# edshkim98/LocalDiffusion-Hallucination

Measured on AMD Instinct MI355X. Metric: local patches/sec (256^2, T=1000), higher is better.
Workload: dtype bf16; 1 GPU; cfg3: 8 local patches (vertical band masks) of one 3x256x256 image per GPU, 4-stage dim-32 conditional UNet (12.1M params), DDPM T=1000, pred_x0, sigmoid schedule; patches_per_gpu=8, parallelism=patch-sharded x1, one all-gather per sample, step_graph_replay=True, whole_batch_graph_flag=False, concurrent_sub_batches=2, weight_split_levels=0

## Files before the change

### include/localdiff_hip.h

```cpp
#ifndef LOCALDIFF_HIP_H
#define LOCALDIFF_HIP_H

#include <stddef.h>
#include <stdint.h>

#ifdef __cplusplus
extern "C" {
#endif

#define LD_OK 0
#define LD_EINVAL (-1)
#define LD_EHIP (-2)
#define LD_ETIMEOUT (-3)

#define LD_F32 0
#define LD_BF16 1
#define LD_F16 2

#define LD_STAT_STRIPES 16

#define LD_ACT_NONE 0
#define LD_ACT_SILU 1
#define LD_ACT_RELU 2

// ... 115 lines not shown
  ld_src a;
  ld_src b;
  int32_t final_act;
  int32_t pool;
  void* out;
  int32_t B, H, W;
  const int32_t* t_ptr;
  int32_t dtype;
} ld_gn_apply_args;
int ld_gn_apply(const ld_gn_apply_args* args, void* stream);

int ld_linattn_kmax(const void* qkv, uint32_t* kmax_enc, int B, int n, int heads, int dim_head,
                    int dtype, void* stream);
int ld_linattn_ctx(const void* qkv, const uint32_t* kmax_enc, float* ctx_part,
                   int B, int n, int heads, int dim_head, int nchunks, int dtype, void* stream);
int ld_linattn_ctx_reduce(const float* ctx_part, int nchunks, float* ctxn, int B, int heads,
                          int dim_head, void* stream);
int ld_linattn_fold(const float* ctxn, const float* w_out ,
                    void* w_packed , int B, int C, int heads, int dim_head,
                    int perm, int dtype, void* stream);
int ld_linattn_ctxfold(const float* ctx_part, int nchunks, const float* w_out ,
                       void* w_packed , int B, int C, int heads, int dim_head,
                       int perm, int dtype, void* stream);
int ld_linattn_kvctx(const void* x, const void* wkv_packed, const float* kshift, float* ctx_part, int B,
                     int n, int C, int heads, int dim_head, int nchunks, int dtype, void* stream);
int ld_linattn_out(const void* x, const void* wq_packed, const float* qshift, const void* mfold,
                   const float* bias, const float* g2, void* out, int B, int n, int C, float q_scale,
                   int dtype, void* stream);
int ld_linattn_kvctx_terms(const void* x, const void* wkv_packed, const float* kshift, float* ctx_part, int B, int n, int C,
                           int heads, int dim_head, int nchunks, int dtype, int weight_terms, void* stream);
int ld_linattn_out_terms(const void* x, const void* wq_packed, const float* qshift, const void* mfold, const float* bias,
                         const float* g2, void* out, int B, int n, int C, float q_scale, int dtype, int weight_terms,
                         void* stream);
size_t ld_linattn_ctx_part_floats(int B, int heads, int dim_head, int nchunks);

int ld_attention(const void* qkv, void* out, int B, int n, int heads, int dim_head, int dtype,
                 void* stream);

int ld_time_mlp(const int32_t* times, int n, const float* freqs, int dim, const float* w1,
                const float* b1, const float* w2, const float* b2, int time_dim, float* temb,
                void* stream);
int ld_time_mlp_fourier(const int32_t* times, int n, const float* weights, int learned_dim, const float* w1,
                        const float* b1, const float* w2, const float* b2, int time_dim, float* temb, void* stream);
int ld_film(const float* temb, int n, int time_dim, const float* w, const float* b, int two_c,
            float* film, void* stream);

int ld_final_conv(const void* x, const float* w , const float* b, float* out_nchw,
                  int B, int H, int W, int Cin, int Cout, int dtype, void* stream);

int ld_final_step(const void* x, const float* w, const float* b, float* model_out, float* x_t, float* x0_out,
                  const float* sched, const int32_t* t_ptr, float lo, float hi, int objective, uint64_t seed,
                  int64_t noise_stream, int B, int H, int W, int Cin, int Cout, int dtype, void* stream);


int ld_final_step_at(const void* x, const float* w, const float* b, float* model_out, float* x_t, float* x0_out,
                     const float* sched, const int32_t* t_ptr, float lo, float hi, int objective, uint64_t seed,
                     int64_t noise_base, int64_t noise_tmul, int64_t noise_first, const float* keep_mask,
                     int B, int H, int W, int Cin, int Cout, int dtype, void* stream);

#define LD_OBJ_X0 0
#define LD_OBJ_NOISE 1
#define LD_OBJ_V 2
#define LD_SCHED_COLS 8
#define LD_SCHED_COEF1 0
#define LD_SCHED_COEF2 1
#define LD_SCHED_SIGMA 2
// ... 131 lines not shown
```

### localdiffusion-hallucination_amd/_cabi.py

```python
import ctypes as C
import os

from .tuning import lib_override_path

_HERE = os.path.dirname(os.path.abspath(__file__))

LIB_PATH = lib_override_path() or os.path.join(_HERE, "csrc", "liblocaldiff_hip.so")

LD_F32, LD_BF16, LD_F16 = 0, 1, 2
ACT_NONE, ACT_SILU, ACT_RELU = 0, 1, 2
EPI_PLAIN, EPI_QKV_LINEAR, EPI_QKV_FULL, EPI_RMS_RES, EPI_RES, EPI_GN_TAIL = 0, 1, 2, 3, 4, 5
OBJ = {"pred_x0": 0, "pred_noise": 1, "pred_v": 2}
SCHED_COLS = 8
STAT_STRIPES = 16
COUNTER_CONV3X3_C32, COUNTER_CONV3X3_GENERIC, COUNTER_CONV3X3_S32 = 0, 1, 2
SEG_SRC_PLAIN, SEG_SRC_POOL, SEG_SRC_CAT_D2S = 0, 1, 2

vp, i32, i64, u64, f32 = C.c_void_p, C.c_int32, C.c_int64, C.c_uint64, C.c_float


class Src(C.Structure):
    _fields_ = [("data", vp), ("C", i32), ("pix_stride", i32), ("upsample", i32), ("gn_stats", vp),
                ("gn_gamma", vp), ("gn_beta", vp), ("gn_groups", i32), ("act", i32), ("film", vp),
                ("film_tstride", i32), ("film_bstride", i32)]
# ... 47 lines not shown
    "ld_memset_bytes": (C.c_int, [vp, C.c_int, C.c_size_t, vp]),
    "ld_event_create": (C.c_int, [C.POINTER(vp)]),
    "ld_event_record": (C.c_int, [vp, vp]),
    "ld_event_elapsed_ms": (C.c_int, [vp, vp, C.POINTER(f32)]),
    "ld_event_destroy": (C.c_int, [vp]),
    "ld_stream_wait_event": (C.c_int, [vp, vp]),
    "ld_counter": (C.c_longlong, [C.c_int]),
    "ld_tuning_set": (C.c_int, [C.c_char_p, C.c_longlong]),
    "ld_tuning_get": (C.c_int, [C.c_char_p, C.POINTER(C.c_longlong)]),
    "ld_tuning_count": (C.c_int, []),
    "ld_tuning_name": (C.c_char_p, [C.c_int]),
    "ld_range_push": (C.c_int, [C.c_char_p]),
    "ld_range_pop": (C.c_int, []),
    "ld_conv3x3": (C.c_int, [C.POINTER(Conv3x3Args), vp]),
    "ld_conv1x1": (C.c_int, [C.POINTER(Conv1x1Args), vp]),
    "ld_pack_conv_weight": (C.c_int, [vp, vp, vp, C.c_int, C.c_int, C.c_int, C.c_int, C.c_int, vp]),
    "ld_pack_conv_weight_terms": (C.c_int, [vp, vp, vp, C.c_int, C.c_int, C.c_int, C.c_int, C.c_int, C.c_int, vp]),
    "ld_conv_image": (C.c_int, [vp, vp, vp, vp, vp, C.c_int, C.c_int, C.c_int, C.c_int, C.c_int,
                                C.c_int, C.c_int, vp]),
    "ld_stem_packed_bytes": (C.c_size_t, []),
    "ld_pack_stem_weight": (C.c_int, [vp, vp, C.c_int, vp]),
    "ld_conv_stem": (C.c_int, [vp, vp, vp, vp, C.c_int, C.c_int, C.c_int, C.c_int, C.c_int, vp]),
    "ld_conv_stem_begin": (C.c_int, [vp, vp, vp, vp, C.c_int, C.c_int, C.c_int, C.c_int, C.c_int, C.POINTER(StepBeginArgs), vp]),
    "ld_gn_apply": (C.c_int, [C.POINTER(GnApplyArgs), vp]),
    "ld_linattn_kmax": (C.c_int, [vp, vp, C.c_int, C.c_int, C.c_int, C.c_int, C.c_int, vp]),
    "ld_linattn_ctx": (C.c_int, [vp, vp, vp, C.c_int, C.c_int, C.c_int, C.c_int, C.c_int, C.c_int, vp]),
    "ld_linattn_ctx_reduce": (C.c_int, [vp, C.c_int, vp, C.c_int, C.c_int, C.c_int, vp]),
    "ld_linattn_fold": (C.c_int, [vp, vp, vp, C.c_int, C.c_int, C.c_int, C.c_int, C.c_int, C.c_int, vp]),
    "ld_linattn_ctxfold": (C.c_int, [vp, C.c_int, vp, vp, C.c_int, C.c_int, C.c_int, C.c_int, C.c_int, C.c_int, vp]),
    "ld_linattn_kvctx": (C.c_int, [vp, vp, vp, vp, C.c_int, C.c_int, C.c_int, C.c_int, C.c_int, C.c_int, C.c_int, vp]),
    "ld_linattn_out": (C.c_int, [vp, vp, vp, vp, vp, vp, vp, C.c_int, C.c_int, C.c_int, f32, C.c_int, vp]),
    "ld_linattn_kvctx_terms": (C.c_int, [vp, vp, vp, vp, C.c_int, C.c_int, C.c_int, C.c_int, C.c_int, C.c_int, C.c_int, C.c_int, vp]),
    "ld_linattn_out_terms": (C.c_int, [vp, vp, vp, vp, vp, vp, vp, C.c_int, C.c_int, C.c_int, f32, C.c_int, C.c_int, vp]),
    "ld_linattn_ctx_part_floats": (C.c_size_t, [C.c_int, C.c_int, C.c_int, C.c_int]),
    "ld_attention": (C.c_int, [vp, vp, C.c_int, C.c_int, C.c_int, C.c_int, C.c_int, vp]),
    "ld_time_mlp": (C.c_int, [vp, C.c_int, vp, C.c_int, vp, vp, vp, vp, C.c_int, vp, vp]),
    "ld_time_mlp_fourier": (C.c_int, [vp, C.c_int, vp, C.c_int, vp, vp, vp, vp, C.c_int, vp, vp]),
    "ld_film": (C.c_int, [vp, C.c_int, C.c_int, vp, vp, C.c_int, vp, vp]),
    "ld_final_conv": (C.c_int, [vp, vp, vp, vp, C.c_int, C.c_int, C.c_int, C.c_int, C.c_int, C.c_int, vp]),
    "ld_final_step": (C.c_int, [vp, vp, vp, vp, vp, vp, vp, vp, f32, f32, C.c_int, u64, i64, C.c_int, C.c_int, C.c_int,
                                C.c_int, C.c_int, C.c_int, vp]),
    "ld_final_step_at": (C.c_int, [vp, vp, vp, vp, vp, vp, vp, vp, f32, f32, C.c_int, u64, i64, i64, i64, vp, C.c_int,
                                   C.c_int, C.c_int, C.c_int, C.c_int, C.c_int, vp]),
    "ld_timing_begin": (C.c_int, [C.c_int]),
    "ld_timing_count": (C.c_int, []),
    "ld_timing_end": (C.c_int, [vp, C.c_int, vp]),
    "ld_timing_end_abs": (C.c_int, [vp, vp, C.c_int, vp]),
    "ld_randn": (C.c_int, [vp, i64, u64, i64, i64, vp, vp]),
    "ld_randn_at": (C.c_int, [vp, i64, i64, u64, i64, i64, vp, vp]),
    "ld_step_add": (C.c_int, [vp, C.c_int, vp]),
    "ld_step_begin": (C.c_int, [vp, C.c_size_t, vp, C.c_size_t, vp, C.c_int, vp, vp, vp]),
    "ld_step_begin_film": (C.c_int, [vp, C.c_size_t, vp, C.c_size_t, vp, C.c_int, vp, vp, vp, C.c_int, vp, vp]),
    "ld_ddim_step_at": (C.c_int, [vp, vp, vp, vp, vp, vp, f32, f32, C.c_int, i64, vp]),
    "ld_ddpm_step": (C.c_int, [vp, vp, vp, vp, vp, vp, vp, f32, f32, C.c_int, i64, vp]),
    "ld_posterior_step": (C.c_int, [vp, vp, vp, vp, vp, vp, i64, vp]),
    "ld_ddim_step": (C.c_int, [vp, vp, vp, vp, f32, f32, f32, f32, f32, f32, f32, f32, f32, C.c_int,
                               C.c_int, i64, vp]),
    "ld_branch_conditions": (C.c_int, [vp, vp, vp, vp, f32, C.c_int, C.c_int, C.c_int, vp]),
    "ld_mask_out": (C.c_int, [vp, vp, f32, C.c_int, C.c_int, C.c_int, vp]),
    "ld_fuse_ddpm": (C.c_int, [vp, vp, vp, vp, vp, vp, vp, f32, f32, C.c_int, C.c_int, C.c_int, vp]),
    "ld_branch_conditions_k": (C.c_int, [vp, vp, vp, f32, C.c_int, C.c_int, C.c_int, C.c_int, vp]),
    "ld_fuse_ddpm_k": (C.c_int, [vp, vp, vp, vp, vp, vp, vp, f32, f32, C.c_int, C.c_int, C.c_int, C.c_int, vp]),
    "ld_fuse_ddim": (C.c_int, [vp, vp, vp, vp, vp, vp, vp, f32, f32, f32, f32, f32, f32, f32, C.c_int,
                               C.c_int, C.c_int, vp]),
    "ld_fuse_ddim_k": (C.c_int, [vp, vp, vp, vp, vp, vp, vp, f32, f32, f32, f32, f32, f32, f32, C.c_int, C.c_int,
                                 C.c_int, C.c_int, vp]),
# ... 85 lines not shown
```

### localdiffusion-hallucination_amd/csrc/linattn_fused.hip

```cpp
#include "common.hip.h"
#include <stdlib.h>

typedef __attribute__((ext_vector_type(4))) short s16x4;

namespace {
constexpr int CTX_STRIDE = 32 * 32 + 64;
constexpr int KTN = 256;
constexpr int PROW = 96;

__device__ __forceinline__ uint2 tr8(const char* p) {
  s16x4 v = __builtin_amdgcn_ds_read_tr16_b64_v4i16((__attribute__((address_space(3))) s16x4*)(const_cast<char*>(p)));
  return __builtin_bit_cast(uint2, v);
}

struct KvCtxArgs {
  const void* x;
  const uint4* wkv;
  float* ctx_part;
  int n, C, heads, nchunks;
  const float* kshift;
  int wsplit;
};
#define KVCTX_PARAMS const void* x_, const uint4* wkv_, float* ctx_part_, int n_, int C_, int heads_, int nchunks_, const float* kshift_, int wsplit_
#define KVCTX_ARGS(a) (a).x, (a).wkv, (a).ctx_part, (a).n, (a).C, (a).heads, (a).nchunks, (a).kshift, (a).wsplit
// ... 469 lines not shown
      for (int m2 = 0; m2 < MT2; ++m2)
        mma16<T>(o[m2], *reinterpret_cast<const uint4*>(s_mf + (s * MT2 + m2) * 1024 + lane * 16), B2[s]);
    float ss = 0.f;
    float y[MT2][4];
#pragma unroll
    for (int m2 = 0; m2 < MT2; ++m2) {
      const float4 bv = bvr[m2];
      y[m2][0] = o[m2][0] + bv.x; y[m2][1] = o[m2][1] + bv.y; y[m2][2] = o[m2][2] + bv.z; y[m2][3] = o[m2][3] + bv.w;
#pragma unroll
      for (int r = 0; r < 4; ++r) ss = fmaf(y[m2][r], y[m2][r], ss);
    }
    ss = kq4_sum(ss);
    const float inv = rms_rinv<false>(ss);
    {
      static_assert(MT2 % 2 == 0, "m-tiles are stored in pairs");
      char* opix = reinterpret_cast<char*>(reinterpret_cast<T*>(a.out) + ((size_t)b * n + (valid ? p : 0)) * C);
#pragma unroll
      for (int m2 = 0; m2 < MT2; m2 += 2) {
        float r4[2][4];
#pragma unroll
        for (int mm = 0; mm < 2; ++mm) {
          const int mq = m2 + mm;
          const float4 gv = gvr[mq];
          float xr[4];
          load4<T>(reinterpret_cast<const T*>(s_x + ((mq >> 1) * 4 + (mq & 1) * 2 + (kq >> 1)) * PLANE + qq * 16 + (kq & 1) * 8), xr);
          r4[mm][0] = y[mq][0] * inv * gv.x + xr[0]; r4[mm][1] = y[mq][1] * inv * gv.y + xr[1];
          r4[mm][2] = y[mq][2] * inv * gv.z + xr[2]; r4[mm][3] = y[mq][3] * inv * gv.w + xr[3];
        }
        const uint4 w16 = pair_frag16<T>(r4[0], r4[1]);
        if (valid) store16_out(opix + m2 * 16 * sizeof(T) + pair_frag16_off(kq), w16);
      }
    }
  }
  }
}

template <typename T>
int kvctx_launch(const KvCtxArgs& a, int B, hipStream_t st) {
  const int nch = a.C / 32, heads = a.heads, nchunks = a.nchunks;
  const float* kshift = a.kshift;
#ifdef LD_DEBUG_VARIANTS
  static const int no_wph = getenv("LD_KVCTX_V1") ? 1 : 0;
#else
  constexpr int no_wph = 0;
#endif
  if (heads == 4 && (!no_wph || kshift)) {
    const size_t lds2 = (size_t)nch * 4 * KTN * 16 + KTN * sizeof(float);
    dim3 grid2(nchunks, B);
    if (a.wsplit) {
      LD_REQUIRE(nch <= 2, "ld_linattn_kvctx: two-term weights are built for C = 32 / 64 (got %d)", a.C);
      if (nch == 1) {
        if (kshift) LD_LAUNCH((kvctx_wph_kernel<T, 1, true, 1>), grid2, dim3(256), lds2, st, KVCTX_ARGS(a));
        else LD_LAUNCH((kvctx_wph_kernel<T, 1, false, 1>), grid2, dim3(256), lds2, st, KVCTX_ARGS(a));
      } else {
        if (kshift) LD_LAUNCH((kvctx_wph_kernel<T, 2, true, 1>), grid2, dim3(256), lds2, st, KVCTX_ARGS(a));
        else LD_LAUNCH((kvctx_wph_kernel<T, 2, false, 1>), grid2, dim3(256), lds2, st, KVCTX_ARGS(a));
      }
    } else if (nch == 1) {
      if (kshift) LD_LAUNCH((kvctx_wph_kernel<T, 1, true>), grid2, dim3(256), lds2, st, KVCTX_ARGS(a));
      else LD_LAUNCH((kvctx_wph_kernel<T, 1, false>), grid2, dim3(256), lds2, st, KVCTX_ARGS(a));
    } else if (nch == 2) {
      if (kshift) LD_LAUNCH((kvctx_wph_kernel<T, 2, true>), grid2, dim3(256), lds2, st, KVCTX_ARGS(a));
      else LD_LAUNCH((kvctx_wph_kernel<T, 2, false>), grid2, dim3(256), lds2, st, KVCTX_ARGS(a));
    } else {
      if (kshift) LD_HIP(ld_allow_lds((kvctx_wph_kernel<T, 4, true>), lds2));
      else LD_HIP(ld_allow_lds((kvctx_wph_kernel<T, 4, false>), lds2));
// ... 9 lines not shown
  if (nch == 1) {
    LD_LAUNCH((kvctx_kernel<T, 1>), grid, dim3(256), lds, st, KVCTX_ARGS(a));
  } else if (nch == 2) {
    LD_HIP(ld_allow_lds((kvctx_kernel<T, 2>), lds));
    LD_LAUNCH((kvctx_kernel<T, 2>), grid, dim3(256), lds, st, KVCTX_ARGS(a));
  } else {
    LD_HIP(ld_allow_lds((kvctx_kernel<T, 4>), lds));
    LD_LAUNCH((kvctx_kernel<T, 4>), grid, dim3(256), lds, st, KVCTX_ARGS(a));
  }
  LD_LAUNCH_CHECK("linattn_kvctx");
  return LD_OK;
}

template <typename T>
int linout_launch(const LinOutArgs& a, int B, hipStream_t st) {
  const int n = a.n, nch = a.C / 32;
  dim3 grid((n + 128 * LINOUT_TPB - 1) / (128 * LINOUT_TPB), B);
  const size_t lds = (size_t)nch * 4 * 128 * 16 + ((size_t)nch << a.wsplit) * 8 * 1024 + (size_t)4 * 2 * nch * 1024 + 128 * sizeof(float);
  if (a.wsplit) {
    LD_REQUIRE(nch <= 2, "ld_linattn_out: two-term weights are built for C = 32 / 64 (got %d)", a.C);
    if (nch == 1) LD_LAUNCH((linout_kernel<T, 1, 1>), grid, dim3(256), lds, st, LINOUT_ARGS(a));
    else LD_LAUNCH((linout_kernel<T, 2, 1>), grid, dim3(256), lds, st, LINOUT_ARGS(a));
  } else if (nch == 1) {
    LD_LAUNCH((linout_kernel<T, 1>), grid, dim3(256), lds, st, LINOUT_ARGS(a));
  } else if (nch == 2) {
    LD_LAUNCH((linout_kernel<T, 2>), grid, dim3(256), lds, st, LINOUT_ARGS(a));
  } else {
    LD_HIP(ld_allow_lds((linout_kernel<T, 4>), lds));
    LD_LAUNCH((linout_kernel<T, 4>), grid, dim3(256), lds, st, LINOUT_ARGS(a));
  }
  LD_LAUNCH_CHECK("linattn_out");
  return LD_OK;
}
}

extern "C" int ld_linattn_kvctx(const void* x, const void* wkv_packed, const float* kshift, float* ctx_part, int B,
                                int n, int C, int heads, int dim_head, int nchunks, int dtype, void* stream) {
  return ld_linattn_kvctx_terms(x, wkv_packed, kshift, ctx_part, B, n, C, heads, dim_head, nchunks, dtype, 1, stream);
}

extern "C" int ld_linattn_kvctx_terms(const void* x, const void* wkv_packed, const float* kshift, float* ctx_part, int B,
                                      int n, int C, int heads, int dim_head, int nchunks, int dtype, int weight_terms,
                                      void* stream) {
  LD_REQUIRE(weight_terms == 1 || weight_terms == 2, "ld_linattn_kvctx: weight_terms %d", weight_terms);
  LD_REQUIRE(x && wkv_packed && ctx_part && B > 0 && n > 0 && nchunks > 0, "ld_linattn_kvctx: bad args");
  LD_REQUIRE(ld_dtype_16(dtype), "ld_linattn_kvctx: 16-bit storage only (fp32 uses the unfused path)");
  LD_REQUIRE(dim_head == 32 && (C == 32 || C == 64 || C == 128), "ld_linattn_kvctx: dim_head 32, C in {32,64,128}");
  LD_REQUIRE(kshift == nullptr || heads == 4, "ld_linattn_kvctx: the single-sweep mode (kshift) needs heads == 4");
  KvCtxArgs a{x, (const uint4*)wkv_packed, ctx_part, n, C, heads, nchunks, kshift, weight_terms == 2 ? 1 : 0};
  hipStream_t st = reinterpret_cast<hipStream_t>(stream);
  return LD_DISPATCH16(dtype, kvctx_launch<T>(a, B, st));
}

extern "C" int ld_linattn_out(const void* x, const void* wq_packed, const float* qshift, const void* mfold,
                              const float* bias, const float* g2, void* out, int B, int n, int C, float q_scale,
                              int dtype, void* stream) {
  return ld_linattn_out_terms(x, wq_packed, qshift, mfold, bias, g2, out, B, n, C, q_scale, dtype, 1, stream);
}

extern "C" int ld_linattn_out_terms(const void* x, const void* wq_packed, const float* qshift, const void* mfold,
                                    const float* bias, const float* g2, void* out, int B, int n, int C, float q_scale,
                                    int dtype, int weight_terms, void* stream) {
  LD_REQUIRE(weight_terms == 1 || weight_terms == 2, "ld_linattn_out: weight_terms %d", weight_terms);
  LD_REQUIRE(x && wq_packed && mfold && bias && g2 && out && B > 0 && n > 0, "ld_linattn_out: bad args");
  LD_REQUIRE(ld_dtype_16(dtype), "ld_linattn_out: 16-bit storage only (fp32 uses the unfused path)");
  LD_REQUIRE(C == 32 || C == 64 || C == 128, "ld_linattn_out: C in {32,64,128}");
  LinOutArgs a{x, (const uint4*)wq_packed, (const uint4*)mfold, bias, g2, out, n, C, q_scale, qshift, weight_terms == 2 ? 1 : 0};
  return LD_DISPATCH16(dtype, linout_launch<T>(a, B, reinterpret_cast<hipStream_t>(stream)));
}
```

### localdiffusion-hallucination_amd/unet.py

```python
import ctypes as C
import math

import numpy as np
import torch
from torch import nn

from . import _cabi as cabi
from .pool import check_declared, intervals_from_declared, peak_live, place_intervals
from .tuning import Tuning
from .weights import UnetConfig, unet_param_shapes

_TORCH_DT = {"fp32": torch.float32, "bf16": torch.bfloat16, "fp16": torch.float16}
_LOWP = ("bf16", "fp16")


def _register(root: nn.Module, dotted: str, tensor: torch.Tensor):
    parts = dotted.split(".")
    mod = root
    for name in parts[:-1]:
        if name not in mod._modules:
            mod.add_module(name, nn.Module())
        mod = mod._modules[name]
    mod.register_parameter(parts[-1], nn.Parameter(tensor, requires_grad=False))


class Unet(nn.Module):
    def __init__(self, dim, init_dim=None, out_dim=None, dim_mults=(1, 2, 4, 8), channels=1,
                 self_condition=False, cond_img=True, resnet_block_groups=8, learned_variance=False,
                 learned_sinusoidal_cond=False, random_fourier_features=False,
                 learned_sinusoidal_dim=16, sinusoidal_pos_emb_theta=10000, attn_dim_head=32,
                 attn_heads=4, full_attn=(False, False, False, True), flash_attn=False, mode="mri",
                 compute_dtype="fp32", tuning=None):
        super().__init__()
        if (learned_sinusoidal_cond or random_fourier_features) and (learned_sinusoidal_dim % 2 or not 2 <= learned_sinusoidal_dim <= 256):
            raise ValueError("learned_sinusoidal_dim must be even (ddpm.py:156) and at most 256")
        if dim != 32:
            raise ValueError("dim must be 32: the conditioning encoder hard-codes its widths "
                             "(unet_model.py:100) and is concatenated with the 8*dim bottleneck")
        if attn_dim_head != 32:
            raise ValueError("attn_dim_head must be 32 (MFMA tile of the attention kernels)")
        if compute_dtype not in _TORCH_DT:
            raise ValueError(f"compute_dtype {compute_dtype!r} (fp32 | bf16 | fp16)")
        full_attn = tuple(full_attn) if isinstance(full_attn, (tuple, list)) else (full_attn,) * len(dim_mults)
        assert len(full_attn) == len(dim_mults)
        init_dim = dim if init_dim is None else init_dim
        learned = bool(learned_sinusoidal_cond or random_fourier_features)
# ... 446 lines not shown
        self._slot_cursor += 1
        assert s < self.stats.shape[0]
        return self.stats[s]

    def t_ptr(self):
        return None

    def src(self, t, c, stride=0, ups=0, gn=None, act=cabi.ACT_NONE, film=None):
        s = cabi.Src()
        s.data, s.C, s.pix_stride, s.upsample = t.data_ptr(), c, stride, ups
        if gn is not None:
            stats, gamma, beta, groups = gn
            s.gn_stats, s.gn_gamma, s.gn_beta, s.gn_groups = stats.data_ptr(), gamma.data_ptr(), beta.data_ptr(), groups
        s.act = act
        if film is not None and self.table_T:
            s.film = self.film_cur.data_ptr() + 4 * self._film_off[id(film)]
            s.film_tstride = s.film_bstride = 0
        elif film is not None:
            s.film = film.data_ptr()
            s.film_tstride = 0
            s.film_bstride = 2 * c
        self.keep.append(t)
        s._tensor = t
        return s

    def _call(self, ops, fn, args, what, meta=None, reads=(), writes=()):
        self.keep.append(args)
        ref = C.byref(args)
        ops.append(lambda st, fn=fn, ref=ref, what=what: cabi.check(fn(ref, st), what))
        if ops is self.ops_main:
            self.meta[len(ops) - 1] = dict(what=what, **(meta or {}))
            self.decl[len(ops) - 1] = ([t for t in reads if t is not None], [t for t in writes if t is not None])

    def _raw(self, ops, fn, what, nbytes=0, flops=0, reads=(), writes=()):
        ops.append(fn)
        if ops is self.ops_main:
            self.meta[len(ops) - 1] = dict(what=what, family=what, bytes=nbytes, flops=flops)
            self.decl[len(ops) - 1] = ([t for t in reads if t is not None], [t for t in writes if t is not None])

    def conv3(self, ops, srcs, wname, cout, h, w, stats=None, groups=8, weight=None, bias=None, addend=None, side=None):
        a = cabi.Conv3x3Args()
        for i, s in enumerate(srcs):
            a.src[i] = s
        a.nsrc = len(srcs)
        weight = self.P["w"][wname + ".weight"] if weight is None else weight
        bias = self.f32[wname + ".bias"] if bias is None else bias
        a.weight, a.bias = weight.data_ptr(), bias.data_ptr()
        a.weight_terms = 2 if weight.data_ptr() in self.P["terms2"] else 1
        a.addend = cabi.ptr(addend)
        self.keep += [weight, bias, addend]
        out = self.buf(h, w, cout)
        a.out = out.data_ptr()
        side_out = None
        if side is not None:
            side_out = self.buf(h, w, cout)
            a.side_weight, a.side_bias, a.side_out = side[0].data_ptr(), side[1].data_ptr(), side_out.data_ptr()
            self.keep += [side[0], side[1]]
        if stats is not None:
            a.out_stats, a.out_groups = stats.data_ptr(), groups
        a.B, a.H, a.W, a.Cout = self.B, h, w, cout
        a.t_ptr = self.t_ptr()
        a.dtype = self.dt
        cin = sum(s.C for s in srcs)
        npx = self.B * h * w
        mt4 = cout % 64 == 0 and ((w + 15) // 16) * ((h + 7) // 8) * (cout // 64) * self.B >= 256
        blocks16 = ((w + 15) // 16) * ((h + 15) // 16) * (cout // (64 if mt4 else 32)) * self.B
        big = blocks16 >= 512 and h >= 16 and not mt4
        big = big or (mt4 and h >= 16 and blocks16 >= self._kt("conv_big4_min"))
        dname = {cabi.LD_F32: "f32", cabi.LD_BF16: "bf16", cabi.LD_F16: "f16"}[self.dt]
        if side is not None:
# ... 115 lines not shown
            act1 = self.gn_apply(ops, n1, None, h, w, cout)
            n1 = self.src(act1, cout)
        raw2 = self.conv3(ops, [n1], p + ".block2.proj", cout, h, w, stats=s2, groups=G)
        n2 = self.src(raw2, cout, gn=(s2, f[p + ".block2.norm.weight"], f[p + ".block2.norm.bias"], G),
                      act=cabi.ACT_SILU)
        if rc is not None:
            out = self.gn_apply(ops, n2, self.src(rc, cout), h, w, cout)
        elif (p + ".res_conv.weight") in f:
            out = self.conv1(ops, srcs_fn(), self.P["w"][p + ".res_conv.weight"], cout, h, w,
                             bias=f[p + ".res_conv.bias"], epi=cabi.EPI_GN_TAIL, gn_tail=n2, what="res_conv+tail " + p)
        else:
            assert res_tensor is not None and cin_total == cout
            out = self.gn_apply(ops, n2, self.src(res_tensor, cout), h, w, cout)
        self.named[p] = out
        return out

    def fusion_block_folded(self, ops, x, c, h, w):
        f, G, p = self.f32, self.cfg.resnet_block_groups, "conv_fusion"
        p1, p2, zero = self.fusion_const
        s1, s2 = self.slot(), self.slot()
        raw1 = self.conv3(ops, [self.src(x, c)], p + ".block1.proj", c, h, w, stats=s1, groups=G,
                          weight=self.P["w"][p + ".block1.proj.weight#x"], bias=zero, addend=p1)
        n1 = self.src(raw1, c, gn=(s1, f[p + ".block1.norm.weight"], f[p + ".block1.norm.bias"], G),
                      act=cabi.ACT_SILU, film=self.films.get(p))
        if self._separate_act(h * w, c):
            n1 = self.src(self.gn_apply(ops, n1, None, h, w, c), c)
        raw2 = self.conv3(ops, [n1], p + ".block2.proj", c, h, w, stats=s2, groups=G)
        n2 = self.src(raw2, c, gn=(s2, f[p + ".block2.norm.weight"], f[p + ".block2.norm.bias"], G), act=cabi.ACT_SILU)
        out = self.conv1(ops, [self.src(x, c)], self.P["w"][p + ".res_conv.weight#x"], c, h, w, bias=None,
                         epi=cabi.EPI_GN_TAIL, gn_tail=n2, residual=p2, what="res_conv+tail " + p)
        self.named[p] = out
        return out

    def linear_attention_fused(self, ops, p, x, c, h, w):
        f, cfg, lib = self.f32, self.cfg, self.lib
        n, hid, B, heads, dt, es = h * w, cfg.hidden, self.B, cfg.attn_heads, self.dt, self.esize
        rule = self.tn.chunk_rule(B)
        chunk_px = rule[0] if n >= 65536 else (rule[1] if n >= 16384 else rule[2])
        nchunks = max(1, min(128, n // chunk_px)) if heads == 4 else max(1, min(32, n // 256))
        if heads == 4 and self.tn.linattn_chunk_px is None:
            while B * nchunks < 512 and nchunks < 512 and n // (2 * nchunks) >= 256:
                nchunks *= 2
        ctx = self._tracked(torch.empty(int(lib.ld_linattn_ctx_part_floats(B, heads, 32, nchunks)), dtype=torch.float32, device=self.dev))
        wfold = self._tracked(torch.empty(B, c * hid, dtype=self.tdt, device=self.dev))
        wout = f[p + ".to_out.0.weight"].reshape(c, hid).contiguous()
        wq, wkv = self.P["wq"][p], self.P["wkv"][p]
        kshift = self.P["kshift"].get(p) if heads == 4 else None
        ksp = kshift.data_ptr() if kshift is not None else None
        qshift = self.P["qshift"].get(p) if heads == 4 else None
        qsp = qshift.data_ptr() if qshift is not None else None
        bias, g2 = f[p + ".to_out.0.bias"], self.P["g2"][p + ".to_out.1.g"]
        out = self.buf(h, w, c)
        self.keep += [ctx, wfold, wout, wq, wkv, kshift, qshift, bias, g2, out, x]
        npx = B * n
        terms = self.P.get("attn_terms", {}).get(p, 1)
        self._raw(ops, lambda st: cabi.check(lib.ld_linattn_kvctx_terms(x.data_ptr(), wkv.data_ptr(), ksp, ctx.data_ptr(), B, n, c,
                                                                        heads, 32, nchunks, dt, terms, st), "linattn_kvctx"),
                  "linattn_kvctx", nbytes=npx * c * es, flops=2 * npx * c * 2 * hid * (1 if kshift is not None else 2) + 2 * npx * hid * 32,
                  reads=[x], writes=[ctx])
        self._raw(ops, lambda st: cabi.check(lib.ld_linattn_ctxfold(ctx.data_ptr(), nchunks, wout.data_ptr(), wfold.data_ptr(), B, c,
                                                                    heads, 32, 1, dt, st), "linattn_ctxfold"),
                  "linattn_ctxfold", nbytes=B * c * hid * es, flops=2 * B * c * hid * 32, reads=[ctx], writes=[wfold])
        scale = cfg.attn_dim_head ** -0.5
        self._raw(ops, lambda st: cabi.check(lib.ld_linattn_out_terms(x.data_ptr(), wq.data_ptr(), qsp, wfold.data_ptr(), bias.data_ptr(),
                                                                      g2.data_ptr(), out.data_ptr(), B, n, c, scale, dt, terms, st),
                                             "linattn_out"),
                  "linattn_out", nbytes=2 * npx * c * es, flops=2 * npx * hid * c * 2, reads=[x, wfold], writes=[out])
        return out

    def linear_attention(self, ops, p, x, c, h, w):
        if self.dt != cabi.LD_F32 and c in (32, 64, 128) and p in self.P["wq"]:
            return self.linear_attention_fused(ops, p, x, c, h, w)
        f, cfg, lib = self.f32, self.cfg, self.lib
        n, hid, B = h * w, cfg.hidden, self.B
        kmax = self.kmax_arena[self._kmax_cursor]
        self._kmax_cursor += 1
        qkv = self.conv1(ops, [self.src(x, c)], self.P["w"][p + ".to_qkv.weight"], 3 * hid, h, w,
                         epi=cabi.EPI_QKV_LINEAR, rms_in=1, what="to_qkv " + p, kmax_out=kmax)
        nchunks = max(1, min(32, n // 256))
        ctx = torch.empty(int(lib.ld_linattn_ctx_part_floats(B, cfg.attn_heads, 32, nchunks)),
                          dtype=torch.float32, device=self.dev)
        wfold = torch.empty(B, c * hid, dtype=self.tdt, device=self.dev)
        wout = f[p + ".to_out.0.weight"].reshape(c, hid).contiguous()
        self.keep += [kmax, ctx, wfold, wout, qkv]
        dt, heads = self.dt, cfg.attn_heads
        es = self.esize
        self._raw(ops, lambda st: cabi.check(lib.ld_linattn_ctx(qkv.data_ptr(), kmax.data_ptr(), ctx.data_ptr(),
                                                                B, n, heads, 32, nchunks, dt, st), "linattn_ctx"),
                  "linattn_ctx", nbytes=2 * B * n * hid * es, flops=2 * B * n * hid * 32, reads=[qkv], writes=[ctx])
        self._raw(ops, lambda st: cabi.check(lib.ld_linattn_ctxfold(ctx.data_ptr(), nchunks, wout.data_ptr(), wfold.data_ptr(),
                                                                    B, c, heads, 32, 0, dt, st), "linattn_ctxfold"),
                  "linattn_ctxfold", nbytes=B * c * hid * es, flops=2 * B * c * hid * 32, reads=[ctx], writes=[wfold])
        q = self.src(qkv, hid, stride=3 * hid)
        return self.conv1(ops, [q], wfold, c, h, w, bias=f[p + ".to_out.0.bias"], epi=cabi.EPI_RMS_RES,
                          bstride=c * hid * self.esize, g2=self.P["g2"][p + ".to_out.1.g"], residual=x,
                          what="lin to_out " + p)
# ... 25 lines not shown
            out = self.buf(h, w, c_out)
            wt, bs = f[wname + ".weight"], f[wname + ".bias"]
            B, dt = self.B, self.dt
            self.keep += [out, wt, bs]
            ops.append(lambda st: cabi.check(lib.ld_conv_image(
                self.cond_in.data_ptr(), wt.data_ptr(), bs.data_ptr(), out.data_ptr(), stats.data_ptr(), G,
                B, cin, h, w, 3, dt, st), "conv_image " + wname))
            return out

        if image:
            a1 = image_conv(p + ".convblock.0", cmid, s1)
            idr = image_conv(p + ".identity.0", cout, s3)
        else:
            a1 = self.conv3(ops, [self.src(x, cin)], p + ".convblock.0", cmid, h, w, stats=s1, groups=G)
            idr = self.conv3(ops, [self.src(x, cin)], p + ".identity.0", cout, h, w, stats=s3, groups=G)
        n1 = self.src(a1, cmid, gn=(s1, f[p + ".convblock.1.weight"], f[p + ".convblock.1.bias"], G),
                      act=cabi.ACT_RELU)
        a2 = self.conv3(ops, [n1], p + ".convblock.3", cout, h, w, stats=s2, groups=G)
        na = self.src(a2, cout, gn=(s2, f[p + ".convblock.4.weight"], f[p + ".convblock.4.bias"], G))
        nb = self.src(idr, cout, gn=(s3, f[p + ".identity.1.weight"], f[p + ".identity.1.bias"], G))
        return self.gn_apply(ops, na, nb, h, w, cout, final_act=cabi.ACT_RELU, pool=1 if pool else 0)

    def _build_cond(self):
        cfg, ops, H, W = self.cfg, self.ops_cond, self.H, self.W
        x = self._basic_block(ops, "cond_model.residual_conv1.0", None, cfg.cond_in_channels, 32, 32, H, W,
                              pool=True, image=True)
        x = self._basic_block(ops, "cond_model.residual_conv2.0", x, 32, 32, 64, H // 2, W // 2, pool=True)
        early = cfg.cond_early_exit
        x = self._basic_block(ops, "cond_model.residual_conv3.0", x, 64, 64, 128, H // 4, W // 4, pool=not early)
        if early:
            return x
        return self._basic_block(ops, "cond_model.mid_conv.0", x, 128, 128, 256, H // 8, W // 8, pool=False)

    def _build_main(self):
        cfg, ops, f, lib, B = self.cfg, self.ops_main, self.f32, self.lib, self.B
        H, W = self.H, self.W
        r = self.buf(H, W, cfg.init_dim)
        wi, bi = f["init_conv.weight"], f["init_conv.bias"]
        if self.dt != cabi.LD_F32 and cfg.init_dim == 32:
            wstem = self.P["stem"]
            self.keep.append(wstem)

            def stem_begin(st, delta, idx_ptr, t_table):
                za, ba, zb, bb = self._begin_args
                rows, row_floats, cur = self._film_args
                g = cabi.StepBeginArgs(za, ba, zb, bb, self._t_dev_ptr, int(delta), idx_ptr, t_table, rows, row_floats, cur)
                cabi.check(lib.ld_conv_stem_begin(self.x_in.data_ptr(), wstem.data_ptr(), bi.data_ptr(), r.data_ptr(), B, cfg.channels,
                                                  H, W, self.dt, C.byref(g), st), "init_conv + step_begin")
            self._stem_begin = stem_begin
            self._raw(ops, lambda st: cabi.check(lib.ld_conv_stem(
                self.x_in.data_ptr(), wstem.data_ptr(), bi.data_ptr(), r.data_ptr(), B, cfg.channels, H, W, self.dt, st),
                "init_conv"), "conv_image7x7",
                nbytes=B * H * W * (4 * cfg.channels + self.esize * cfg.init_dim), flops=2 * 49 * cfg.channels * cfg.init_dim * B * H * W, writes=[r])
        else:
            self._raw(ops, lambda st: cabi.check(lib.ld_conv_image(
                self.x_in.data_ptr(), wi.data_ptr(), bi.data_ptr(), r.data_ptr(), None, 1, B, cfg.channels, H, W, 7,
                self.dt, st), "init_conv"), "conv_image7x7",
                nbytes=B * H * W * (4 * cfg.channels + self.esize * cfg.init_dim), flops=2 * 49 * cfg.channels * cfg.init_dim * B * H * W, writes=[r])
        self.named["init_conv"] = r
        x, c, h, w = r, cfg.init_dim, H, W
        skips = []
        io, n = cfg.in_out, len(cfg.in_out)
        for i, (cin, cout) in enumerate(io):
            p = f"downs.{i}"
            x = self.resnet_block(ops, p + ".0", lambda x=x, c=c: [self.src(x, c)], c, c, h, w, res_tensor=x)
            skips.append((x, c))
            x = self.resnet_block(ops, p + ".1", lambda x=x, c=c: [self.src(x, c)], c, c, h, w, res_tensor=x)
            x = self.attention(ops, p + ".2", x, c, h, w, cfg.full_attn[i])
            skips.append((x, c))
            if i < n - 1:
                h, w = h // 2, w // 2
                x = self.conv1(ops, [self.src(x, c)], self.P["w"][p + ".3.1.weight"], cout, h, w,
                               bias=f[p + ".3.1.bias"], unshuffle=1, what="downsample " + p)
            else:
                x = self.conv3(ops, [self.src(x, c)], p + ".3", cout, h, w)
            self.named[p + ".3"] = x
            c = cout
        x = self.resnet_block(ops, "mid_block1", lambda x=x, c=c: [self.src(x, c)], c, c, h, w, res_tensor=x)
        x = self.attention(ops, "mid_attn", x, c, h, w, True)
        x = self.resnet_block(ops, "mid_block2", lambda x=x, c=c: [self.src(x, c)], c, c, h, w, res_tensor=x)
        feat = self.cond_feat
        if self.fusion_const is not None:
            x = self.fusion_block_folded(ops, x, c, h, w)
        else:
            x = self.resnet_block(ops, "conv_fusion", lambda x=x, c=c: [self.src(x, c), self.src(feat, c)], 2 * c, c, h, w)
        for j, ((cin, cout), full) in enumerate(zip(reversed(io), reversed(cfg.full_attn))):
            p = f"ups.{j}"
            for k in (0, 1):
                sk, sc = skips.pop()
                x = self.resnet_block(ops, f"{p}.{k}", lambda x=x, c=c, sk=sk, sc=sc: [self.src(x, c), self.src(sk, sc)],
                                      c + sc, cout, h, w)
                c = cout
            x = self.attention(ops, p + ".2", x, c, h, w, full)
            if j < n - 1:
                h, w = h * 2, w * 2
                x = self.conv3(ops, [self.src(x, c, ups=1)], p + ".3.1", cin, h, w)
            else:
                x = self.conv3(ops, [self.src(x, c)], p + ".3", cin, h, w)
            self.named[p + ".3"] = x
            c = cin
        if self.tn.recompute_stem and self._track is not None and self.dt != cabi.LD_F32 and cfg.init_dim == 32:
            r2 = self.buf(H, W, cfg.init_dim)
            wstem2 = self.P["stem"]
# ... 109 lines not shown
```

Measured before the change: 6.668 patches/s.

## Fuse linear-attention output with following pixel-unshuffle downsample conv

Adds a HIP kernel that computes the linear-attention output (q projection, softmax, folded context, RMSNorm, residual) and then, from the same LDS tile of 2x64 pixels, runs the 1x1 downsample conv over the unshuffled 2x2 neighbourhood. The UNet builder routes eligible down levels (linear attention, matching channel pairs, single-term weights) through this fused path. This is meant to remove one kernel launch per level and the global re-read of the attention output by the separate downsample conv. In exchange it uses more LDS and registers per block, and blocks are tied to 2-row tiles, which may reduce occupancy.

```diff
diff --git a/include/localdiff_hip.h b/include/localdiff_hip.h
--- a/include/localdiff_hip.h
+++ b/include/localdiff_hip.h
@@ -171,6 +171,9 @@
 int ld_linattn_out_terms(const void* x, const void* wq_packed, const float* qshift, const void* mfold, const float* bias,
                          const float* g2, void* out, int B, int n, int C, float q_scale, int dtype, int weight_terms,
                          void* stream);
+int ld_linattn_out_down(const void* x, const void* wq_packed, const float* qshift, const void* mfold, const float* bias,
+                        const float* g2, void* out, const void* wd_packed, const float* bd, void* dout, int B, int H, int W,
+                        int C, int Cd, float q_scale, int dtype, void* stream);
 size_t ld_linattn_ctx_part_floats(int B, int heads, int dim_head, int nchunks);
 
 int ld_attention(const void* qkv, void* out, int B, int n, int heads, int dim_head, int dtype,
diff --git a/localdiffusion-hallucination_amd/_cabi.py b/localdiffusion-hallucination_amd/_cabi.py
--- a/localdiffusion-hallucination_amd/_cabi.py
+++ b/localdiffusion-hallucination_amd/_cabi.py
@@ -103,6 +103,8 @@
     "ld_linattn_out": (C.c_int, [vp, vp, vp, vp, vp, vp, vp, C.c_int, C.c_int, C.c_int, f32, C.c_int, vp]),
     "ld_linattn_kvctx_terms": (C.c_int, [vp, vp, vp, vp, C.c_int, C.c_int, C.c_int, C.c_int, C.c_int, C.c_int, C.c_int, C.c_int, vp]),
     "ld_linattn_out_terms": (C.c_int, [vp, vp, vp, vp, vp, vp, vp, C.c_int, C.c_int, C.c_int, f32, C.c_int, C.c_int, vp]),
+    "ld_linattn_out_down": (C.c_int, [vp, vp, vp, vp, vp, vp, vp, vp, vp, vp, C.c_int, C.c_int, C.c_int, C.c_int, C.c_int, f32,
+                                      C.c_int, vp]),
     "ld_linattn_ctx_part_floats": (C.c_size_t, [C.c_int, C.c_int, C.c_int, C.c_int]),
     "ld_attention": (C.c_int, [vp, vp, C.c_int, C.c_int, C.c_int, C.c_int, C.c_int, vp]),
     "ld_time_mlp": (C.c_int, [vp, C.c_int, vp, C.c_int, vp, vp, vp, vp, C.c_int, vp, vp]),
diff --git a/localdiffusion-hallucination_amd/csrc/linattn_fused.hip b/localdiffusion-hallucination_amd/csrc/linattn_fused.hip
--- a/localdiffusion-hallucination_amd/csrc/linattn_fused.hip
+++ b/localdiffusion-hallucination_amd/csrc/linattn_fused.hip
@@ -525,6 +525,189 @@
       }
     }
   }
+  }
+}
+
+template <typename T, int NCH, int MTD>
+__global__ __launch_bounds__(256) void linout_down_kernel(LINOUT_PARAMS, const uint4* wd_, const float* bd_, void* dout_, int W_) {
+  const LinOutArgs a{x_, wq_, mfold_, bias_, g2_, out_, n_, C_, q_scale_, qshift_, wsplit_};
+  constexpr int NW = 2, NPT = 64 * NW, PLANE = NPT * 16, MT2 = 2 * NCH;
+  constexpr int NCD = 4 * NCH, CD = 16 * MTD;
+  static_assert(MTD % 2 == 0, "downsample m-tiles are stored in pairs");
+  extern __shared__ __attribute__((aligned(16))) char smem[];
+  char* s_x = smem;
+  char* s_wq = s_x + NCH * 4 * PLANE;
+  char* s_mf = s_wq + NCH * 8 * 1024;
+  float* s_rinv = reinterpret_cast<float*>(s_mf + 4 * MT2 * 1024);
+  char* s_wd = reinterpret_cast<char*>(s_rinv + NPT);
+  float* s_bd = reinterpret_cast<float*>(s_wd + NCD * MTD * 1024);
+  const int b = blockIdx.y;
+  const int tid = threadIdx.x, lane = tid & 63, wv = tid >> 6, li = lane & 15, kq = lane >> 4;
+  const int n = a.n, C = a.C, W = W_;
+  const T* xb = reinterpret_cast<const T*>(a.x) + (size_t)b * n * C;
+  const int tpr = W >> 6;
+  const int ty = blockIdx.x / tpr, y0 = 2 * ty, x0 = 64 * (blockIdx.x - ty * tpr);
+  auto pix = [&](int qq) { return (y0 + (qq >> 6)) * W + x0 + (qq & 63); };
+  constexpr int WQ_IT = NCH * 8 * 64 / 256, MF_IT = 4 * MT2 * 64 / 256;
+  const uint4* mf = a.mfold + (size_t)b * 4 * MT2 * 64;
+  u32x4 wq_r[WQ_IT], mf_r[MF_IT];
+  u32x4 x_r[NCH][NW];
+#pragma unroll
+  for (int i = 0; i < WQ_IT; ++i) wq_r[i] = *reinterpret_cast<const u32x4*>(a.wq + tid + i * 256);
+#pragma unroll
+  for (int i = 0; i < MF_IT; ++i) mf_r[i] = *reinterpret_cast<const u32x4*>(mf + tid + i * 256);
+#pragma unroll
+  for (int c = 0; c < NCH; ++c)
+#pragma unroll
+    for (int it = 0; it < NW; ++it)
+      x_r[c][it] = *reinterpret_cast<const u32x4*>(xb + (size_t)pix((it * 4 + wv) * 16 + li) * C + c * 32 + kq * 8);
+  float4 bvr[MT2], gvr[MT2];
+#pragma unroll
+  for (int m2 = 0; m2 < MT2; ++m2) {
+    bvr[m2] = *reinterpret_cast<const float4*>(a.bias + m2 * 16 + kq * 4);
+    gvr[m2] = *reinterpret_cast<const float4*>(a.g2 + m2 * 16 + kq * 4);
+  }
+  const float4 qsv = *reinterpret_cast<const float4*>(reinterpret_cast<const char*>(a.qshift ? a.qshift : a.bias) + (lane & 0));
+  float4 bdv = make_float4(0.f, 0.f, 0.f, 0.f);
+  if (tid < CD / 4) bdv = *reinterpret_cast<const float4*>(bd_ + tid * 4);
+  {
+    const int wvu = __builtin_amdgcn_readfirstlane(wv);
+#pragma unroll
+    for (int i = 0; i < NCD * MTD / 4; ++i)
+      glds16(wd_ + (size_t)(i * 4 + wvu) * 64 + lane, __builtin_amdgcn_readfirstlane(lds_addr(s_wd + (i * 4 + wvu) * 1024)));
+  }
+  __builtin_amdgcn_sched_barrier(0);
+  const float qs2[4] = {qsv.x * 1.4426950408889634f, qsv.y * 1.4426950408889634f, qsv.z * 1.4426950408889634f, qsv.w * 1.4426950408889634f};
+#pragma unroll
+  for (int i = 0; i < WQ_IT; ++i) *reinterpret_cast<u32x4*>(s_wq + (tid + i * 256) * 16) = wq_r[i];
+#pragma unroll
+  for (int i = 0; i < MF_IT; ++i) *reinterpret_cast<u32x4*>(s_mf + (tid + i * 256) * 16) = mf_r[i];
+  float rs[NW];
+#pragma unroll
+  for (int i = 0; i < NW; ++i) rs[i] = 0.f;
+#pragma unroll
+  for (int c = 0; c < NCH; ++c)
+#pragma unroll
+    for (int it = 0; it < NW; ++it) {
+      const int qq = (it * 4 + wv) * 16 + li;
+      const uint4 raw = make_uint4(x_r[c][it][0], x_r[c][it][1], x_r[c][it][2], x_r[c][it][3]);
+      float v[8];
+      unpack16<T>(raw, v);
+#pragma unroll
+      for (int e = 0; e < 8; ++e) rs[it] = fmaf(v[e], v[e], rs[it]);
+      *reinterpret_cast<uint4*>(s_x + (c * 4 + kq) * PLANE + qq * 16) = raw;
+    }
+#pragma unroll
+  for (int it = 0; it < NW; ++it) {
+    float r = rs[it];
+    r = kq4_sum(r);
+    if (kq == 0) s_rinv[(it * 4 + wv) * 16 + li] = rms_rinv<false>(r);
+  }
+  if (tid < CD / 4) *reinterpret_cast<float4*>(s_bd + tid * 4) = bdv;
+  __builtin_amdgcn_s_waitcnt(0x0F70);
+  __syncthreads();
+#pragma unroll
+  for (int j = 0; j < NW; ++j) {
+    const int qq = (wv * NW + j) * 16 + li, p = pix(qq);
+    f32x4 q[8];
+#pragma unroll
+    for (int m = 0; m < 8; ++m) q[m] = f32x4{0.f, 0.f, 0.f, 0.f};
+#pragma unroll
+    for (int c = 0; c < NCH; ++c) {
+      const uint4 Bf = *reinterpret_cast<const uint4*>(s_x + (c * 4 + kq) * PLANE + qq * 16);
+#pragma unroll
+      for (int m = 0; m < 8; ++m)
+        mma16<T>(q[m], *reinterpret_cast<const uint4*>(s_wq + (c * 8 + m) * 1024 + lane * 16), Bf);
+    }
+    const float rinv2 = s_rinv[qq] * 1.4426950408889634f;
+    uint4 B2[4];
+#pragma unroll
+    for (int hh = 0; hh < 4; ++hh) {
+      float v0[4], v1[4];
+      float mx;
+      if (a.qshift) {
+        mx = qs2[hh];
+      } else {
+        mx = -INFINITY;
+#pragma unroll
+        for (int r = 0; r < 4; ++r) mx = fmaxf(mx, fmaxf(q[2 * hh][r], q[2 * hh + 1][r]) * rinv2);
+        mx = kq4_max(mx);
+      }
+      float sum = 0.f;
+#pragma unroll
+      for (int r = 0; r < 4; ++r) {
+        v0[r] = __builtin_amdgcn_exp2f(fmaf(q[2 * hh][r], rinv2, -mx)); v1[r] = __builtin_amdgcn_exp2f(fmaf(q[2 * hh + 1][r], rinv2, -mx));
+        sum += v0[r] + v1[r];
+      }
+      sum = kq4_sum(sum);
+      const float sc = a.q_scale * __builtin_amdgcn_rcpf(sum);
+      B2[hh] = make_uint4(pack2<T>(v0[0] * sc, v0[1] * sc), pack2<T>(v0[2] * sc, v0[3] * sc),
+                          pack2<T>(v1[0] * sc, v1[1] * sc), pack2<T>(v1[2] * sc, v1[3] * sc));
+    }
+    f32x4 o[MT2];
+#pragma unroll
+    for (int m2 = 0; m2 < MT2; ++m2) o[m2] = f32x4{0.f, 0.f, 0.f, 0.f};
+#pragma unroll
+    for (int s = 0; s < 4; ++s)
+#pragma unroll
+      for (int m2 = 0; m2 < MT2; ++m2)
+        mma16<T>(o[m2], *reinterpret_cast<const uint4*>(s_mf + (s * MT2 + m2) * 1024 + lane * 16), B2[s]);
+    float ss = 0.f;
+    float y[MT2][4];
+#pragma unroll
+    for (int m2 = 0; m2 < MT2; ++m2) {
+      const float4 bv = bvr[m2];
+      y[m2][0] = o[m2][0] + bv.x; y[m2][1] = o[m2][1] + bv.y; y[m2][2] = o[m2][2] + bv.z; y[m2][3] = o[m2][3] + bv.w;
+#pragma unroll
+      for (int r = 0; r < 4; ++r) ss = fmaf(y[m2][r], y[m2][r], ss);
+    }
+    ss = kq4_sum(ss);
+    const float inv = rms_rinv<false>(ss);
+    char* opix = reinterpret_cast<char*>(reinterpret_cast<T*>(a.out) + ((size_t)b * n + p) * C);
+    uint4 w16s[MT2 / 2];
+#pragma unroll
+    for (int m2 = 0; m2 < MT2; m2 += 2) {
+      float r4[2][4];
+#pragma unroll
+      for (int mm = 0; mm < 2; ++mm) {
+        const int mq = m2 + mm;
+        const float4 gv = gvr[mq];
+        float xr[4];
+        load4<T>(reinterpret_cast<const T*>(s_x + ((mq >> 1) * 4 + (mq & 1) * 2 + (kq >> 1)) * PLANE + qq * 16 + (kq & 1) * 8), xr);
+        r4[mm][0] = y[mq][0] * inv * gv.x + xr[0]; r4[mm][1] = y[mq][1] * inv * gv.y + xr[1];
+        r4[mm][2] = y[mq][2] * inv * gv.z + xr[2]; r4[mm][3] = y[mq][3] * inv * gv.w + xr[3];
+      }
+      w16s[m2 / 2] = pair_frag16<T>(r4[0], r4[1]);
+      store16_out(opix + m2 * 16 * sizeof(T) + pair_frag16_off(kq), w16s[m2 / 2]);
+    }
+    asm volatile("" ::: "memory");
+    const int g = (kq & 1) * 2 + (kq >> 1);
+#pragma unroll
+    for (int c = 0; c < NCH; ++c) *reinterpret_cast<uint4*>(s_x + (c * 4 + g) * PLANE + qq * 16) = w16s[c];
+  }
+  __syncthreads();
+  T* dbase = reinterpret_cast<T*>(dout_) + ((size_t)b * (n >> 2) + (size_t)ty * (W >> 1) + (x0 >> 1)) * CD;
+#pragma unroll
+  for (int u = wv; u < MTD; u += 4) {
+    const int j = u & 1, mp = u >> 1;
+    f32x4 acc[2] = {f32x4{0.f, 0.f, 0.f, 0.f}, f32x4{0.f, 0.f, 0.f, 0.f}};
+#pragma unroll
+    for (int ch = 0; ch < NCD; ++ch) {
+      const int pp = ch / NCH, cc = ch % NCH;
+      const int t = (pp >> 1) * 64 + 2 * (j * 16 + li) + (pp & 1);
+      const uint4 Bf = *reinterpret_cast<const uint4*>(s_x + (cc * 4 + kq) * PLANE + t * 16);
+#pragma unroll
+      for (int mm = 0; mm < 2; ++mm)
+        mma16<T>(acc[mm], *reinterpret_cast<const uint4*>(s_wd + (ch * MTD + 2 * mp + mm) * 1024 + lane * 16), Bf);
+    }
+    float v[2][4];
+#pragma unroll
+    for (int mm = 0; mm < 2; ++mm) {
+      const float4 bv = *reinterpret_cast<const float4*>(s_bd + (2 * mp + mm) * 16 + kq * 4);
+      v[mm][0] = acc[mm][0] + bv.x; v[mm][1] = acc[mm][1] + bv.y; v[mm][2] = acc[mm][2] + bv.z; v[mm][3] = acc[mm][3] + bv.w;
+    }
+    const uint4 w16 = pair_frag16<T>(v[0], v[1]);
+    store16_out(reinterpret_cast<char*>(dbase + (size_t)(j * 16 + li) * CD + 2 * mp * 16) + pair_frag16_off(kq), w16);
   }
 }
 
@@ -600,6 +783,36 @@
   LD_LAUNCH_CHECK("linattn_out");
   return LD_OK;
 }
+
+struct LinDownArgs {
+  const uint4* wd;
+  const float* bd;
+  void* dout;
+  int W;
+};
+
+template <typename T>
+int linout_down_launch(const LinOutArgs& a, const LinDownArgs& d, int B, int cd, hipStream_t st) {
+  const int nch = a.C / 32, mtd = cd / 16;
+  dim3 grid(a.n / 128, B);
+  const size_t lds = (size_t)nch * 4 * 128 * 16 + (size_t)nch * 8 * 1024 + (size_t)4 * 2 * nch * 1024 + 128 * sizeof(float) +
+                     (size_t)4 * nch * mtd * 1024 + (size_t)cd * sizeof(float);
+#define LD_LD_ARGS LINOUT_ARGS(a), d.wd, d.bd, d.dout, d.W
+  if (nch == 1 && mtd == 2) {
+    LD_LAUNCH((linout_down_kernel<T, 1, 2>), grid, dim3(256), lds, st, LD_LD_ARGS);
+  } else if (nch == 1 && mtd == 4) {
+    LD_LAUNCH((linout_down_kernel<T, 1, 4>), grid, dim3(256), lds, st, LD_LD_ARGS);
+  } else if (nch == 2 && mtd == 4) {
+    LD_HIP(ld_allow_lds((linout_down_kernel<T, 2, 4>), lds));
+    LD_LAUNCH((linout_down_kernel<T, 2, 4>), grid, dim3(256), lds, st, LD_LD_ARGS);
+  } else {
+    LD_HIP(ld_allow_lds((linout_down_kernel<T, 2, 8>), lds));
+    LD_LAUNCH((linout_down_kernel<T, 2, 8>), grid, dim3(256), lds, st, LD_LD_ARGS);
+  }
+#undef LD_LD_ARGS
+  LD_LAUNCH_CHECK("linattn_out_down");
+  return LD_OK;
+}
 }
 
 extern "C" int ld_linattn_kvctx(const void* x, const void* wkv_packed, const float* kshift, float* ctx_part, int B,
@@ -636,3 +849,20 @@
   LinOutArgs a{x, (const uint4*)wq_packed, (const uint4*)mfold, bias, g2, out, n, C, q_scale, qshift, weight_terms == 2 ? 1 : 0};
   return LD_DISPATCH16(dtype, linout_launch<T>(a, B, reinterpret_cast<hipStream_t>(stream)));
 }
+
+extern "C" int ld_linattn_out_down(const void* x, const void* wq_packed, const float* qshift, const void* mfold,
+                                   const float* bias, const float* g2, void* out, const void* wd_packed, const float* bd,
+                                   void* dout, int B, int H, int W, int C, int Cd, float q_scale, int dtype, void* stream) {
+  LD_REQUIRE(x && wq_packed && mfold && bias && g2 && out && wd_packed && bd && dout && B > 0 && H > 0 && W > 0,
+             "ld_linattn_out_down: bad args");
+  LD_REQUIRE(ld_dtype_16(dtype), "ld_linattn_out_down: 16-bit storage only");
+  LD_REQUIRE(W % 64 == 0 && H % 2 == 0, "ld_linattn_out_down: needs W %% 64 == 0 and even H (got %dx%d)", H, W);
+  LD_REQUIRE((C == 32 && (Cd == 32 || Cd == 64)) || (C == 64 && (Cd == 64 || Cd == 128)),
+             "ld_linattn_out_down: C -> Cd in {32 -> 32, 32 -> 64, 64 -> 64, 64 -> 128} (got %d -> %d)", C, Cd);
+  LD_REQUIRE((reinterpret_cast<uintptr_t>(bd) & 15) == 0 && (reinterpret_cast<uintptr_t>(wd_packed) & 15) == 0,
+             "ld_linattn_out_down: downsample weights / bias must be 16-byte aligned");
+  LD_REQUIRE((long)H * W < (1L << 31), "ld_linattn_out_down: image too large");
+  LinOutArgs a{x, (const uint4*)wq_packed, (const uint4*)mfold, bias, g2, out, H * W, C, q_scale, qshift, 0};
+  const LinDownArgs d{(const uint4*)wd_packed, bd, dout, W};
+  return LD_DISPATCH16(dtype, linout_down_launch<T>(a, d, B, Cd, reinterpret_cast<hipStream_t>(stream)));
+}
diff --git a/localdiffusion-hallucination_amd/unet.py b/localdiffusion-hallucination_amd/unet.py
--- a/localdiffusion-hallucination_amd/unet.py
+++ b/localdiffusion-hallucination_amd/unet.py
@@ -12,6 +12,7 @@
 
 _TORCH_DT = {"fp32": torch.float32, "bf16": torch.bfloat16, "fp16": torch.float16}
 _LOWP = ("bf16", "fp16")
+DOWN_FOLD_LEVELS = (0, 1, 2)
 
 
 def _register(root: nn.Module, dotted: str, tensor: torch.Tensor):
@@ -524,10 +525,10 @@
             self.meta[len(ops) - 1] = dict(what=what, **(meta or {}))
             self.decl[len(ops) - 1] = ([t for t in reads if t is not None], [t for t in writes if t is not None])
 
-    def _raw(self, ops, fn, what, nbytes=0, flops=0, reads=(), writes=()):
+    def _raw(self, ops, fn, what, nbytes=0, flops=0, reads=(), writes=(), family=None):
         ops.append(fn)
         if ops is self.ops_main:
-            self.meta[len(ops) - 1] = dict(what=what, family=what, bytes=nbytes, flops=flops)
+            self.meta[len(ops) - 1] = dict(what=what, family=family or what, bytes=nbytes, flops=flops)
             self.decl[len(ops) - 1] = ([t for t in reads if t is not None], [t for t in writes if t is not None])
 
     def conv3(self, ops, srcs, wname, cout, h, w, stats=None, groups=8, weight=None, bias=None, addend=None, side=None):
@@ -709,7 +710,7 @@
         self.named[p] = out
         return out
 
-    def linear_attention_fused(self, ops, p, x, c, h, w):
+    def linear_attention_fused(self, ops, p, x, c, h, w, down=None):
         f, cfg, lib = self.f32, self.cfg, self.lib
         n, hid, B, heads, dt, es = h * w, cfg.hidden, self.B, cfg.attn_heads, self.dt, self.esize
         rule = self.tn.chunk_rule(B)
@@ -739,6 +740,19 @@
                                                                     heads, 32, 1, dt, st), "linattn_ctxfold"),
                   "linattn_ctxfold", nbytes=B * c * hid * es, flops=2 * B * c * hid * 32, reads=[ctx], writes=[wfold])
         scale = cfg.attn_dim_head ** -0.5
+        if down is not None:
+            wd, bd, cd = down
+            dout = self.buf(h // 2, w // 2, cd)
+            self.keep += [wd, bd, dout]
+            d_el = npx * c + npx // 4 * cd + 4 * c * cd
+            self._raw(ops, lambda st: cabi.check(lib.ld_linattn_out_down(x.data_ptr(), wq.data_ptr(), qsp, wfold.data_ptr(), bias.data_ptr(),
+                                                                         g2.data_ptr(), out.data_ptr(), wd.data_ptr(), bd.data_ptr(),
+                                                                         dout.data_ptr(), B, h, w, c, cd, scale, dt, st),
+                                                 "linattn_out_down"),
+                      "linattn_out + downsample " + p[:-len(".2")], nbytes=2 * npx * c * es + d_el * es,
+                      flops=2 * npx * hid * c * 2 + 2 * 4 * c * cd * (npx // 4), reads=[x, wfold], writes=[out, dout],
+                      family="linattn_out_down")
+            return out, dout
         self._raw(ops, lambda st: cabi.check(lib.ld_linattn_out_terms(x.data_ptr(), wq.data_ptr(), qsp, wfold.data_ptr(), bias.data_ptr(),
                                                                       g2.data_ptr(), out.data_ptr(), B, n, c, scale, dt, terms, st),
                                              "linattn_out"),
@@ -830,6 +844,13 @@
             return x
         return self._basic_block(ops, "cond_model.mid_conv.0", x, 128, 128, 256, H // 8, W // 8, pool=False)
 
+    def _folds_downsample(self, i, c, cout, h, w):
+        p = f"downs.{i}"
+        return (i in DOWN_FOLD_LEVELS and self.dt != cabi.LD_F32 and not self.cfg.full_attn[i] and p + ".2" in self.P["wq"]
+                and (c, cout) in ((32, 32), (32, 64), (64, 64), (64, 128)) and h % 2 == 0 and w % 64 == 0
+                and self.P.get("attn_terms", {}).get(p + ".2", 1) == 1
+                and self.P["w"][p + ".3.1.weight"].data_ptr() not in self.P["terms2"])
+
     def _build_main(self):
         cfg, ops, f, lib, B = self.cfg, self.ops_main, self.f32, self.lib, self.B
         H, W = self.H, self.W
@@ -864,9 +885,18 @@
             x = self.resnet_block(ops, p + ".0", lambda x=x, c=c: [self.src(x, c)], c, c, h, w, res_tensor=x)
             skips.append((x, c))
             x = self.resnet_block(ops, p + ".1", lambda x=x, c=c: [self.src(x, c)], c, c, h, w, res_tensor=x)
-            x = self.attention(ops, p + ".2", x, c, h, w, cfg.full_attn[i])
+            fold = i < n - 1 and self._folds_downsample(i, c, cout, h, w)
+            if fold:
+                x, xd = self.linear_attention_fused(ops, p + ".2", x, c, h, w,
+                                                    down=(self.P["w"][p + ".3.1.weight"], f[p + ".3.1.bias"], cout))
+                self.named[p + ".2"] = x
+            else:
+                x = self.attention(ops, p + ".2", x, c, h, w, cfg.full_attn[i])
             skips.append((x, c))
-            if i < n - 1:
+            if fold:
+                h, w = h // 2, w // 2
+                x = xd
+            elif i < n - 1:
                 h, w = h // 2, w // 2
                 x = self.conv1(ops, [self.src(x, c)], self.P["w"][p + ".3.1.weight"], cout, h, w,
                                bias=f[p + ".3.1.bias"], unshuffle=1, what="downsample " + p)
```

Result: no change. 6.778 patches/s (median of 6 runs) (+1.7%).
